# ishine/Test-time-adaptation-ASR-SUTA

Measured on AMD Instinct MI355X. Metric: adapted utterances/sec (whole node) at 10 SUTA steps, w2v2-base; WER parity, higher is better.
Workload: dtype f32; 1 GPU; wav2vec2-base SUTA 10 steps on 128000-sample (8 s) utterances, 164 utterances per GPU per step, scripts/LS.sh flags; model=wav2vec2-base, global_batch=164, seq_len=399, n_samples=128000, suta_steps=10, parallelism=utterance-sharded x1

## Files before the change

test-time-adaptation-asr-suta_amd/config.py:

```python
from __future__ import annotations

import copy
import json
import os
from typing import List

_BASE = dict(
    hidden_size=768, num_hidden_layers=12, num_attention_heads=12, intermediate_size=3072,
    vocab_size=32, conv_dim=[512] * 7, conv_kernel=[10, 3, 3, 3, 3, 2, 2], conv_stride=[5, 2, 2, 2, 2, 2, 2],
    conv_bias=False, feat_extract_norm="group", do_stable_layer_norm=False,
    num_conv_pos_embeddings=128, num_conv_pos_embedding_groups=16, layer_norm_eps=1e-5,
)

_LARGE = dict(_BASE, hidden_size=1024, num_hidden_layers=24, num_attention_heads=16, intermediate_size=4096,
              conv_bias=True, feat_extract_norm="layer", do_stable_layer_norm=True)

_XLSR_1B = dict(_LARGE, hidden_size=1280, num_hidden_layers=48, num_attention_heads=16, intermediate_size=5120)
_XLSR_2B = dict(_LARGE, hidden_size=1920, num_hidden_layers=48, num_attention_heads=16, intermediate_size=7680)

_TINY_GROUP = dict(_BASE, hidden_size=64, num_hidden_layers=2, num_attention_heads=4, intermediate_size=128,
                   conv_dim=[32] * 7, num_conv_pos_embeddings=16, num_conv_pos_embedding_groups=4)
_TINY_LAYER = dict(_TINY_GROUP, conv_bias=True, feat_extract_norm="layer", do_stable_layer_norm=True)
_TINY_HD80 = dict(_TINY_LAYER, hidden_size=160, num_attention_heads=2, num_conv_pos_embedding_groups=2,
                  intermediate_size=320)
_TINY_HD120 = dict(_TINY_HD80, hidden_size=240)

PRESETS = {
    "facebook/wav2vec2-base-960h": _BASE,
    "wav2vec2-base": _BASE,
    "facebook/wav2vec2-large-960h-lv60": _LARGE,
    "facebook/wav2vec2-large-960h-lv60-self": _LARGE,
    "wav2vec2-large": _LARGE,
    "facebook/wav2vec2-xls-r-1b": _XLSR_1B,
    "wav2vec2-xls-r-1b": _XLSR_1B,
    "facebook/wav2vec2-xls-r-2b": _XLSR_2B,
    "wav2vec2-xls-r-2b": _XLSR_2B,
    "tiny-group": _TINY_GROUP,
    "tiny-layer": _TINY_LAYER,
    "tiny-hd80": _TINY_HD80,
    "tiny-hd120": _TINY_HD120,
}


def head_dim(cfg: dict) -> int:
    return cfg["hidden_size"] // cfg["num_attention_heads"]


def flash_attention_applies(cfg: dict) -> bool:
    d = head_dim(cfg)
    return d == 64 or (64 < d <= 128 and d % 8 == 0)


def get_config(name_or_path: str) -> dict:
    if name_or_path in PRESETS:
        return copy.deepcopy(PRESETS[name_or_path])
    cfg_file = os.path.join(name_or_path, "config.json")
    if os.path.isfile(cfg_file):
        with open(cfg_file) as f:
            raw = json.load(f)
        cfg = copy.deepcopy(_BASE)
        for k in cfg:
            if k in raw:
                cfg[k] = raw[k]
        return cfg
    raise KeyError(f"unknown model '{name_or_path}': not a preset and no config.json found")


def frame_lengths(cfg: dict, n_samples: int) -> List[int]:
    out, L = [], int(n_samples)
    for k, s in zip(cfg["conv_kernel"], cfg["conv_stride"]):
        L = (L - k) // s + 1
        out.append(L)
    return out


def num_frames(cfg: dict, n_samples: int) -> int:
    return frame_lengths(cfg, n_samples)[-1]


def param_shapes(cfg: dict):
    H, C = cfg["hidden_size"], cfg["conv_dim"]
    out = [("wav2vec2.masked_spec_embed", (H,))]
    group = cfg["feat_extract_norm"] == "group"
    for i, (c, k) in enumerate(zip(C, cfg["conv_kernel"])):
        cin = 1 if i == 0 else C[i - 1]
        b = f"wav2vec2.feature_extractor.conv_layers.{i}."
        out.append((b + "conv.weight", (c, cin, k)))
        if cfg["conv_bias"]:
            out.append((b + "conv.bias", (c,)))
        if (group and i == 0) or not group:
            out += [(b + "layer_norm.weight", (c,)), (b + "layer_norm.bias", (c,))]
    fp = "wav2vec2.feature_projection."
    out += [(fp + "layer_norm.weight", (C[-1],)), (fp + "layer_norm.bias", (C[-1],)),
# ... 20 lines not shown
```

test-time-adaptation-asr-suta_amd/csrc/common.h:

```cpp
#pragma once
#include <hip/hip_runtime.h>
#include <stdint.h>
#include <string>

#define SUTA_WAVE 64

typedef float f32x4 __attribute__((ext_vector_type(4)));
typedef float f32x16 __attribute__((ext_vector_type(16)));

__device__ __forceinline__ float gelu_f(float x) {
    return 0.5f * x * (1.0f + erff(x * 0.70710678118654752f));
}
__device__ __forceinline__ float dgelu_f(float x) {
    const float cdf = 0.5f * (1.0f + erff(x * 0.70710678118654752f));
    const float pdf = 0.39894228040143268f * __expf(-0.5f * x * x);
    return cdf + x * pdf;
}

__device__ __forceinline__ float erfc_t(float z, float t, float ez2) {
    float p = 0.17087277f;
    p = fmaf(p, t, -0.82215223f);
    p = fmaf(p, t, 1.48851587f);
    p = fmaf(p, t, -1.13520398f);
    p = fmaf(p, t, 0.27886807f);
    p = fmaf(p, t, -0.18628806f);
    p = fmaf(p, t, 0.09678418f);
    p = fmaf(p, t, 0.37409196f);
    p = fmaf(p, t, 1.00002368f);
    p = fmaf(p, t, -1.26551223f);
    return t * ez2 * __expf(p);
}
__device__ __forceinline__ float gelu_fast(float x) {
    const float z = fabsf(x) * 0.70710678118654752f;
    const float t = __builtin_amdgcn_rcpf(fmaf(0.5f, z, 1.0f));
    const float erfc = erfc_t(z, t, __expf(-z * z));
    return 0.5f * x * (x >= 0.f ? 2.0f - erfc : erfc);
}
__device__ __forceinline__ float dgelu_fast(float x) {
    const float z = fabsf(x) * 0.70710678118654752f;
    const float t = __builtin_amdgcn_rcpf(fmaf(0.5f, z, 1.0f));
    const float e = __expf(-z * z);
    const float erfc = erfc_t(z, t, e);
    const float cdf = 0.5f * (x >= 0.f ? 2.0f - erfc : erfc);
    return cdf + x * (0.39894228040143268f * e);
}

struct SutaSwitches {
    int latched;
    int fast_gelu;
    int flash_fwd_plane;
    int flash_bwd_plane;
    int flash_bf16_img;
    int conv_planes;
    int pre_bf16;
    int conv_z_bf16;
    int dy_planes;
    int conv_dx_planes;
    int fused_conv_ln;
    int flash_fwd_nw;
    int hbx;
    int splitk;
    int hbx_form;
    int ln_rpw;
    int hbx_dbg;
    int fused_delta;
    int hbx_t;
    int hbp_conv;
    int hbt4;
    int epi_fast;
    int loss_wide;
    int f32p;
    int sdpl_wide;
};
void suta_latch_switches();
void set_max_lds_once(const void* fn, size_t bytes, const char* name);
const SutaSwitches& suta_switches();

typedef float f32x2v __attribute__((ext_vector_type(2)));
__device__ __forceinline__ f32x2v phi_as2(f32x2v x, f32x2v& q) {
    const f32x2v z = __builtin_elementwise_abs(x) * 0.70710678118654752f;
    f32x2v p = z * 0.0000430638f + 0.0002765672f;
    p = p * z + 0.0001520143f;
    p = p * z + 0.0092705272f;
    p = p * z + 0.0422820123f;
    p = p * z + 0.0705230784f;
    p = p * z + 1.0f;
    p = p * p;
    p = p * p;
    p = p * p;
    p = p * p;
    q = f32x2v{__builtin_amdgcn_rcpf(p.x), __builtin_amdgcn_rcpf(p.y)};
    const f32x2v h = 0.5f * q;
    return f32x2v{x.x >= 0.f ? 1.0f - h.x : h.x, x.y >= 0.f ? 1.0f - h.y : h.y};
}
__device__ __forceinline__ f32x2v gelu2_bf16ep(f32x2v x) {
    f32x2v q;
    return x * phi_as2(x, q);
}
__device__ __forceinline__ f32x2v dgelu2_bf16ep(f32x2v x) {
    f32x2v q;
    const f32x2v cdf = phi_as2(x, q);
    const f32x2v a = x * x * (-0.5f * 1.4426950408889634f);
    const f32x2v e = f32x2v{__builtin_amdgcn_exp2f(a.x), __builtin_amdgcn_exp2f(a.y)};
    return cdf + (x * 0.39894228040143268f) * e;
}

__device__ __forceinline__ float wave_sum(float v) {
#pragma unroll
    for (int o = 32; o > 0; o >>= 1) v += __shfl_xor(v, o, 64);
    return v;
}
__device__ __forceinline__ double wave_sum_d(double v) {
#pragma unroll
    for (int o = 32; o > 0; o >>= 1) v += __shfl_xor(v, o, 64);
    return v;
}
__device__ __forceinline__ float wave_max(float v) {
#pragma unroll
    for (int o = 32; o > 0; o >>= 1) v = fmaxf(v, __shfl_xor(v, o, 64));
    return v;
}

enum {
    EPI_BIAS = 1,
    EPI_GELU = 2,
// ... 16 lines not shown
    long sA0, sA1, sB0, sB1, sC0, sC1;
    int ta, tb;
    int segK, pad, Mvalid;
    int segB;
    long sBseg;
    const float* bias;
    long sBias0, sBias1;
    const float* R;
    long ldr, sR0, sR1;
    const float* aux;
    long ldaux, sAux0, sAux1;
    float* C2;
    long ldc2, sC20, sC21;
    const float* rowv;
    long sRow0, sRow1;
    const int* zrows;
    const int* zmvalid;
    float alpha;
    int epi;
    int splits, kchunk;
    float* ws;
    int va, vb;
    int mode;
    int order;
    const void* Ab;
    const void* Bb;
    long ldab, ldbb;
    void* Cb;
    long ldcb;
    long sCb1;
    int off32;
    int preb;
    int fgelu;
    const float* dlt_o;
    long ldo;
    float* delta;
    int dT, dNH;
};

void gemm_init(GemmParams& p);
bool gemm_hbx_t_selected(const GemmParams& p);
void gemm_launch(GemmParams p, hipStream_t st, float* ws, long ws_floats);
void gemm_set_variant(int tile, int nbuf);
void gemm_set_mode(int mode);
bool gemm_run_hb_class(const GemmParams& p, dim3 grid, hipStream_t st);
void launch_to_bf16(const float* src, long lds, long rows, int K, void* dst, hipStream_t st);
void launch_transpose_bf16(const float* src, long zs, int Z, int K, int N, void* dst, hipStream_t st,
                          void* dstn = nullptr);
int gemm_get_mode();
void gemm_census_enable(bool on);
std::string gemm_census_text();
bool gemm_census_is_on();
void gemm_census_time(const std::string& shape, double ms);
```

test-time-adaptation-asr-suta_amd/csrc/gemm.hip:

```cpp
#include "gemm_kernels.h"
#include <algorithm>
#include <cstdio>
#include <cstdlib>
#include <atomic>
#include <map>
#include <mutex>
#include <stdexcept>
#include <string>

namespace {

bool aligned16(const void* q) { return (reinterpret_cast<uintptr_t>(q) & 15) == 0; }

int g_force_tile = -1;
int g_nbuf = 3;
int g_mode = 0;

}

void gemm_set_variant(int tile, int nbuf) {
    g_force_tile = tile;
    g_nbuf = nbuf;
}

static std::mutex g_census_mu;
static std::map<std::string, long> g_census;
static std::atomic<bool> g_census_on{false};
static std::map<std::string, std::pair<double, long>> g_census_ms;

void gemm_census_enable(bool on) {
    std::lock_guard<std::mutex> lk(g_census_mu);
    g_census_on = on;
    g_census.clear();
    g_census_ms.clear();
}

bool gemm_census_is_on() { return g_census_on; }

void gemm_census_time(const std::string& shape, double ms) {
    std::lock_guard<std::mutex> lk(g_census_mu);
    auto& e = g_census_ms[shape];
    e.first += ms;
    e.second += 1;
}

std::string gemm_census_text() {
    std::lock_guard<std::mutex> lk(g_census_mu);
    std::string out;
    for (const auto& kv : g_census) out += kv.first + " " + std::to_string(kv.second) + "\n";
    for (const auto& kv : g_census_ms)
        out += "ms|" + kv.first + "|n=" + std::to_string(kv.second.second) + " " +
               std::to_string((long)(kv.second.first * 1000.0)) + "\n";
    return out;
}

static void census(const char* kernel, int BM, int BN, const GemmParams& p, int splits) {
    if (!g_census_on) return;
    char key[160], gkey[160], ekey[96];
    snprintf(key, sizeof key, "%s %dx%d z=%ld split=%d %s%s%s", kernel, BM, BN, (long)p.Z, splits, p.ta ? "T" : "N",
             p.tb ? "T" : "N", p.segK > 0 ? (p.segB ? " conv-seg" : " conv") : "");
    snprintf(gkey, sizeof gkey, "grid %s %dx%d gx=%d gy=%d z=%ld split=%d", kernel, BM, BN, (p.N + BN - 1) / BN,
             (p.M + BM - 1) / BM, (long)p.Z, splits);
    snprintf(ekey, sizeof ekey, "epi %s %dx%d %d", kernel, BM, BN, p.epi);
    std::lock_guard<std::mutex> lk(g_census_mu);
    ++g_census[key];
    ++g_census[gkey];
    ++g_census[ekey];
}

void gemm_set_mode(int mode) { g_mode = mode; }
int gemm_get_mode() { return g_mode; }

void gemm_init(GemmParams& p) {
    p = GemmParams{};
    p.Z = 1;
    p.zdiv = 1;
    p.alpha = 1.f;
    p.splits = 1;
    p.mode = g_mode;
}

static int choose_tile(long M, long N, long Z, long K, int mode) {
    struct Cand {
        int bm, bn;
        double eff;
    };
    static const Cand glds[4] = {{128, 128, 1.0}, {128, 64, 0.93}, {64, 128, 0.92}, {64, 64, 0.85}};
    static const Cand x6[4] = {{128, 128, 1.0}, {128, 64, 0.9}, {64, 128, 0.9}, {64, 64, 0.75}};
    const Cand* cands = mode == 0 ? glds : x6;
    int best = 0;
    double bt = 1e300;
    for (int c = 0; c < 4; ++c) {
        const long tiles = ((M + cands[c].bm - 1) / cands[c].bm) * ((N + cands[c].bn - 1) / cands[c].bn) * Z;
        const double area = (double)cands[c].bm * cands[c].bn;
        const double t = std::max((double)tiles, 256.0) * area / cands[c].eff;
        if (t < bt * 0.999) {
// ... 221 lines not shown
```

test-time-adaptation-asr-suta_amd/csrc/ops.h:

```cpp
#pragma once
#include "common.h"

void launch_wave_normalize(const float* x, float* y, int B, long N, const int* lens, hipStream_t st);

void launch_conv0(const float* x, long N, const float* W, const float* bias, long wstride, float* z, int B, int L0,
                  int C, int K, int S, hipStream_t st, void* zb = nullptr);

void launch_front_gn_fwd(const float* x, long N, const float* W, const float* bias, long wstride, int B, int L0, int C,
                         int K, int S, const float* g, const float* beta, float* mean, float* rstd, float* a,
                         double* dpart, const int* L0s, hipStream_t st);
void launch_front_gn_bwd(const float* x, long N, const float* W, const float* bias, long wstride, int B, int L0, int C,
                         int K, int S, const float* g, const float* beta, const float* mean, const float* rstd,
                         float* da, float* dgamma, float* dbeta, float* dW, long gstride, double* dpart, float* fpart,
                         const int* L0s, hipStream_t st);

void launch_layernorm_fwd(const float* x, const float* g, const float* beta, long pstride, int rows_per_utt,
                          float* y, float* xhat, float* rstd, int rows, int D, float eps, int gelu_out,
                          hipStream_t st, void* yb = nullptr, float* mean = nullptr, const void* xb = nullptr);
void launch_layernorm_bwd(const float* dy, const float* xhat, const float* rstd, const float* g, const float* beta,
                          long pstride, int rows_per_utt, int B, int D, int gelu_in, const float* post_aux,
                          const float* resid, float* dx, float* dgamma, float* dbeta, long gstride, float* part,
                          hipStream_t st, void* dxb = nullptr, const float* x = nullptr, const float* mean = nullptr,
                          const void* dyb = nullptr);

long layernorm_bwd_conv_part_floats(int B, int rows_per_utt, int D, int ktaps);
bool launch_layernorm_bwd_conv(const float* dy, const float* rstd, const float* g, const float* beta, long pstride,
                               int rows_per_utt, int B, int D, float* dx, float* dgamma, float* dbeta, float* dbias,
                               float* dw, long gstride, float* part, hipStream_t st, const float* x, const float* mean,
                               const float* xw, long xws, int xs, int ktaps, void* dxb = nullptr, int bf16_in = 0);
void launch_colsum(const float* x, int B, int rows, int C, float* out, long ostride, float* part, hipStream_t st);

bool flash_dh_ok(int dh);
long flash_dq_scratch_floats(int B, int T, int NH, int dh);
bool flash_fwd_reads_plane(bool bf16, const void* qkvb, int H, int dh);
bool flash_bwd_reads_planes(bool bf16, const void* qkvb, const void* dctxb, int H, int dh);
bool launch_flash_fwd(const float* qkv, float* ctx, float* lse, int B, int T, int NH, int H, int dh, float scale,
                      const int* tlen, bool bf16, hipStream_t st, void* ctxb = nullptr, const void* qkvb = nullptr);
bool launch_flash_bwd(const float* qkv, const float* dctx, const float* lse, const float* delta, float* dqkv,
                      float* dqp, int B, int T, int NH, int H, int dh, float scale, const int* tlen, bool bf16,
                      hipStream_t st, void* dqkvb = nullptr, const void* qkvb = nullptr,
                      const void* dctxb = nullptr);
bool flash_wide_dh(int dh);
long flash_wide_dq_scratch_floats(int B, int T, int NH, int dh);
bool launch_flash_wide_fwd(const float* qkv, float* ctx, float* lse, int B, int T, int NH, int H, int dh, float scale,
                           const int* tlen, bool bf16, hipStream_t st, void* ctxb);
bool launch_flash_wide_bwd(const float* qkv, const float* dctx, const float* lse, const float* delta, float* dqkv,
                           float* dqp, int B, int T, int NH, int H, int dh, float scale, const int* tlen, bool bf16,
                           hipStream_t st, void* dqkvb);
bool launch_posconv(bool fwd, const float* x, const float* W, const float* bias, const float* R, float* C, float* C2,
                    int B, int T, int H, int G, int K, int pad, const int* tlen, hipStream_t st);
bool launch_posconv_bf16(bool fwd, const float* x, const void* Wt, const float* bias, const float* R, float* C,
                         float* C2, int B, int T, int H, int G, int K, int pad, const int* tlen, hipStream_t st);
void launch_softmax_rows(float* s, long nrows, int T, long ld, const int* tlen, long rows_per_utt, hipStream_t st);

void launch_attn_delta(const float* dO, const float* O, float* delta, int B, int T, int NH, int dh, hipStream_t st);

void launch_dgelu_mul(const float* g, const float* z, float* out, long n, hipStream_t st);

struct LossHP {
    float temp, em_coef, div_coef;
    int reweight, non_blank;
};
#define SUTA_MAX_VOCAB 1024
size_t suta_loss_scratch_floats(int B, long T, int V);
void launch_suta_loss(const float* logits, int B, int T, int V, LossHP hp, const int* tlen, float* dlogits, float* loss,
                      float* scratch, hipStream_t st);

enum { SDPL_KIND_NORMAL = 0, SDPL_KIND_DROP = 1, SDPL_KIND_SPACE = 2, SDPL_KIND_FAIL = 3 };
enum { SDPL_FLAG_LOOKUP = 1, SDPL_FLAG_INFEASIBLE = 2 };
struct SdplTable {
    const int* off;
    const int* ids;
    const int* kind;
    int space_id;
};
long sdpl_scratch_floats(int T, int V);
void launch_sdpl_loss(const float* logits, int B, int T, int V, float pl_coef, const int* tlen, float* dlogits,
                      float* loss, float* scratch, int* err, const SdplTable* tab, hipStream_t st);

void launch_argmax(const float* logits, long rows, int V, int* ids, hipStream_t st);

struct AdamRun {
    long start, len;
    int k;
};
#define SUTA_MAX_RUNS 24
#define ADAM_TAB 52
struct AdamArgs {
    int nruns;
    AdamRun runs[SUTA_MAX_RUNS];
    int blk0[SUTA_MAX_RUNS];
    float beta1, beta2, omb1, omb2, eps, lr_wd;
    int sgd;
    float step_size[5][5];
    float bc2_sqrt[5][5];
    const float* tab;
    const int* step;
};
void launch_broadcast(float* dst, const float* src, long n, int B, hipStream_t st);
void launch_step_advance(int* step, hipStream_t st);
void launch_adam(float* P, const float* G, float* M, float* V, long pstride, int B, const AdamArgs& a,
                 hipStream_t st);
```

test-time-adaptation-asr-suta_amd/csrc/ops.hip:

```cpp
#include "ops.h"
#include <algorithm>
#include <map>
#include <mutex>
#include <stdexcept>
#include <string>

namespace {

inline int cdiv(long a, long b) { return (int)((a + b - 1) / b); }

template <typename T>
__device__ __forceinline__ T block_sum(T v, T* red) {
    const int lane = threadIdx.x & 63, w = threadIdx.x >> 6;
#pragma unroll
    for (int o = 32; o > 0; o >>= 1) v += __shfl_xor(v, o, 64);
    __syncthreads();
    if (lane == 0) red[w] = v;
    __syncthreads();
    T s = red[0] + red[1] + red[2] + red[3];
    __syncthreads();
    return s;
}

__global__ __launch_bounds__(256) void wave_normalize_kernel(const float* __restrict__ x, float* __restrict__ y,
                                                             long N, const int* __restrict__ lens) {
    __shared__ double red[4];
    const float* xb = x + (long)blockIdx.x * N;
    float* yb = y + (long)blockIdx.x * N;
    const long n = lens ? lens[blockIdx.x] : N;
    double s = 0.0;
    for (long i = threadIdx.x; i < n; i += 256) s += xb[i];
    s = block_sum(s, red);
    const double mean = s / (double)n;
    double q = 0.0;
    for (long i = threadIdx.x; i < n; i += 256) {
        const double d = (double)xb[i] - mean;
        q += d * d;
    }
    q = block_sum(q, red);
    const float meanf = (float)mean;
    const float denom = (float)sqrt(q / (double)n + 1e-7);
    for (long i = threadIdx.x; i < N; i += 256) yb[i] = i < n ? (xb[i] - meanf) / denom : 0.f;
}

constexpr int C0_ROWS = 32;
__global__ __launch_bounds__(256) void conv0_kernel(const float* __restrict__ x, long N, const float* __restrict__ W,
                                                    const float* __restrict__ bias, long wstride,
                                                    float* __restrict__ z, int L0, int C, int K, int S) {
    __shared__ float xs[C0_ROWS * 16 + 16];
    const int b = blockIdx.y;
    const int t0 = blockIdx.x * C0_ROWS;
    const float* xb = x + (long)b * N;
    const float* Wb = W + (long)b * wstride;
    const float* bb = bias ? bias + (long)b * wstride : nullptr;
    const int nx = (C0_ROWS - 1) * S + K;
    for (int i = threadIdx.x; i < nx; i += 256) {
        const long gi = (long)t0 * S + i;
        xs[i] = gi < N ? xb[gi] : 0.f;
// ... 778 lines not shown
                const int row = (it * 4) / CG, col = (it * 4) % CG;
                *reinterpret_cast<f32x4*>(dst + row * WS + col) = st[n];
            }
        }
    };
    f32x4 acc[NC];
#pragma unroll
    for (int nf = 0; nf < NC; ++nf) acc[nf] = f32x4{0.f, 0.f, 0.f, 0.f};
    const int nch = K / CHT;
    load_chunk(0);
    store_chunk(0);
    __syncthreads();
    const float* arow = win + (16 * w + r) * XS + g;
    for (int c = 0; c < nch; ++c) {
        if (c + 1 < nch) load_chunk(c + 1);
        const float* wb = wbuf + (c & 1) * (CHT * CG * WS) + g * WS + r;
#pragma unroll
        for (int qq = 0; qq < CHT; ++qq) {
            const float* ap = arow + (c * CHT + qq) * XS;
            const float* bp = wb + qq * CG * WS;
#pragma unroll
            for (int j = 0; j < CG / 4; ++j) {
                const float a = ap[4 * j];
                float b[NC];
#pragma unroll
                for (int nf = 0; nf < NC; ++nf) b[nf] = bp[4 * j * WS + 16 * nf];
#pragma unroll
                for (int nf = 0; nf < NC; ++nf) acc[nf] = __builtin_amdgcn_mfma_f32_16x16x4f32(a, b[nf], acc[nf], 0, 0, 0);
            }
        }
        if (c + 1 < nch) store_chunk((c + 1) & 1);
        __syncthreads();
    }
#pragma unroll
    for (int i = 0; i < 4; ++i) {
        const int t = t0 + 16 * w + 4 * g + i;
        if (t >= T) continue;
        const long o = ((long)u * T + t) * H + gi * CG;
#pragma unroll
        for (int nf = 0; nf < NC; ++nf) {
            const int co = 16 * nf + r;
            float v;
            if (FWD) {
                v = acc[nf][i] * 1.0f + bias[gi * CG + co];
                C2[o + co] = v;
                v = gelu_f(v) + R[o + co];
            } else {
                v = acc[nf][i] + R[o + co];
                if (tlen && t >= tl) v = 0.f;
            }
            C[o + co] = v;
        }
    }
}

constexpr int PCB_CHT = 4;
constexpr int PCB_RS = 72;
template <int WB, bool FWD>
__global__ __launch_bounds__(WB * 64, 1) void posconv_bf16_kernel(const float* __restrict__ x,
                                                                  const __bf16* __restrict__ Wt,
                                                                  const float* __restrict__ bias,
                                                                  const float* __restrict__ R, float* __restrict__ C,
                                                                  float* __restrict__ C2, int T, int H, int G, int K,
                                                                  int pad, const int* __restrict__ tlen, int ntile,
                                                                  int nutt) {
    constexpr int CG = 64, NT = WB * 64, WROWS = 32 * WB;
    constexpr int CHUNK = PCB_CHT * CG * CG / 8;
    constexpr int LPT = (CHUNK + NT - 1) / NT;
    extern __shared__ __attribute__((aligned(16))) __bf16 pcb_smem[];
    __bf16* win = pcb_smem;
    __bf16* wbuf = pcb_smem + (WROWS + K - 1) * PCB_RS;
    typedef __bf16 b8 __attribute__((ext_vector_type(8)));
    typedef __bf16 b4 __attribute__((ext_vector_type(4)));

    const int nb = gridDim.x;
    int L = blockIdx.x;
    if ((nb & 7) == 0) L = (L & 7) * (nb >> 3) + (L >> 3);
    const int tile = L % ntile;
    const int u = (L / ntile) % nutt;
    const int gi = L / (ntile * nutt);
    const int t0 = tile * WROWS;
    const int tl = tlen ? tlen[u] : T;
    const int w = threadIdx.x >> 6, lane = threadIdx.x & 63, l32 = lane & 31, h = lane >> 5;
    const float* xb = x + (long)u * T * H + gi * CG;
    const __bf16* wg = Wt + (long)gi * K * CG * CG;

    const int nwin = (WROWS + K - 1) * (CG / 4);
    for (int it = threadIdx.x; it < nwin; it += NT) {
        const int row = it / (CG / 4), c4 = (it % (CG / 4)) * 4;
        const int t = t0 - pad + row;
        f32x4 v = {0.f, 0.f, 0.f, 0.f};
        if (t >= 0 && t < tl) v = *reinterpret_cast<const f32x4*>(xb + (long)t * H + c4);
        b4 o;
#pragma unroll
        for (int e = 0; e < 4; ++e) o[e] = (__bf16)v[e];
        *reinterpret_cast<b4*>(win + row * PCB_RS + c4) = o;
    }
    b8 st[LPT];
    auto load_chunk = [&](int c) {
        const b8* src = reinterpret_cast<const b8*>(wg + (long)c * PCB_CHT * CG * CG);
#pragma unroll
        for (int n = 0; n < LPT; ++n) {
            const int it = threadIdx.x + n * NT;
            if (it < CHUNK) st[n] = src[it];
        }
    };
// ... 944 lines not shown
#undef LBC
    const int nvec = 3 + ktaps;
    hipLaunchKernelGGL(chunk_reduce_conv, dim3(cdiv(D, 256), B, nvec), dim3(256), 0, st, part, nchunk, nvec, D, dgamma,
                       dbeta, dbias, dw, gstride);
    return true;
}

void launch_colsum(const float* x, int B, int rows, int C, float* out, long ostride, float* part, hipStream_t st) {
    const int nchunk = cdiv(rows, CS_ROWS);
    hipLaunchKernelGGL(colsum_partial, dim3(nchunk, B), dim3(256), 0, st, x, rows, C, part, nchunk);
    hipLaunchKernelGGL(chunk_reduce, dim3(cdiv(C, 256), B), dim3(256), 0, st, part, nchunk, 1, C, out, (float*)nullptr,
                       ostride);
}

void launch_softmax_rows(float* s, long nrows, int T, long ld, const int* tlen, long rows_per_utt, hipStream_t st) {
    dim3 grid((unsigned)((nrows + 3) / 4));
    if (T <= 256) hipLaunchKernelGGL(softmax_rows_kernel<4>, grid, dim3(256), 0, st, s, nrows, T, ld, tlen,
                                    rows_per_utt);
    else if (T <= 512) hipLaunchKernelGGL(softmax_rows_kernel<8>, grid, dim3(256), 0, st, s, nrows, T, ld, tlen,
                                    rows_per_utt);
    else if (T <= 1024) hipLaunchKernelGGL(softmax_rows_kernel<16>, grid, dim3(256), 0, st, s, nrows, T, ld, tlen,
                                    rows_per_utt);
    else hipLaunchKernelGGL(softmax_rows_kernel<32>, grid, dim3(256), 0, st, s, nrows, T, ld, tlen,
                                    rows_per_utt);
}

constexpr int PC_CHT = 2;
#define HIPCHK_OPS(x)                                                                        \
    do {                                                                                     \
        if ((x) != hipSuccess) throw std::runtime_error("hipFuncSetAttribute(posconv) failed"); \
    } while (0)

template <int CG, bool FWD>
static void posconv_go(int WB, dim3 grid, size_t lds, hipStream_t st, const float* x, const float* W,
                       const float* bias, const float* R, float* C, float* C2, int T, int H, int G, int K, int pad,
                       const int* tlen, int ntile, int B) {
#define PC(WB_)                                                                                                   \
    do {                                                                                                          \
        set_max_lds_once(reinterpret_cast<const void*>(&posconv_kernel<CG, WB_, PC_CHT, FWD>), 160 * 1024,       \
                         "posconv_kernel");                                                                       \
        hipLaunchKernelGGL((posconv_kernel<CG, WB_, PC_CHT, FWD>), grid, dim3(WB_ * 64), lds, st, x, W, bias, R, C, \
                           C2, T, H, G, K, pad, tlen, ntile, B);                                                  \
    } while (0)
    switch (WB) {
        case 4: PC(4); break;
        case 5: PC(5); break;
        case 6: PC(6); break;
        case 7: PC(7); break;
        default: PC(8); break;
    }
#undef PC
}

bool launch_posconv(bool fwd, const float* x, const float* W, const float* bias, const float* R, float* C, float* C2,
                    int B, int T, int H, int G, int K, int pad, const int* tlen, hipStream_t st) {
    const int CG = H / G;
    if ((CG != 48 && CG != 64) || K % PC_CHT || H % 4) return false;
    int WB = 8;
    long best = 1L << 40;
    for (int wb = 8; wb >= 4; --wb) {
        const long tiles = (T + 16 * wb - 1) / (16 * wb);
        const long waste = tiles * 16 * wb - T;
        if (waste < best) {
            best = waste;
            WB = wb;
        }
    }
    const int ntile = (T + 16 * WB - 1) / (16 * WB);
    const int XS = CG + 4, WS = (CG % 64 == 0) ? CG + 16 : CG;
    const size_t lds = ((size_t)(16 * WB + K - 1) * XS + 2 * PC_CHT * CG * WS) * sizeof(float);
    if (lds > 160 * 1024) return false;
    const dim3 grid((unsigned)((long)G * B * ntile));
    if (CG == 48) {
        if (fwd) posconv_go<48, true>(WB, grid, lds, st, x, W, bias, R, C, C2, T, H, G, K, pad, tlen, ntile, B);
        else posconv_go<48, false>(WB, grid, lds, st, x, W, bias, R, C, C2, T, H, G, K, pad, tlen, ntile, B);
    } else {
        if (fwd) posconv_go<64, true>(WB, grid, lds, st, x, W, bias, R, C, C2, T, H, G, K, pad, tlen, ntile, B);
        else posconv_go<64, false>(WB, grid, lds, st, x, W, bias, R, C, C2, T, H, G, K, pad, tlen, ntile, B);
    }
    return true;
}

template <bool FWD>
static void posconv_bf16_go(int WB, dim3 grid, size_t lds, hipStream_t st, const float* x, const __bf16* W,
                            const float* bias, const float* R, float* C, float* C2, int T, int H, int G, int K, int pad,
                            const int* tlen, int ntile, int B) {
#define PCB(WB_)                                                                                                  \
    do {                                                                                                          \
        set_max_lds_once(reinterpret_cast<const void*>(&posconv_bf16_kernel<WB_, FWD>), 160 * 1024,              \
                         "posconv_bf16_kernel");                                                                  \
        hipLaunchKernelGGL((posconv_bf16_kernel<WB_, FWD>), grid, dim3(WB_ * 64), lds, st, x, W, bias, R, C, C2, T, \
                           H, G, K, pad, tlen, ntile, B);                                                         \
    } while (0)
    switch (WB) {
        case 4: PCB(4); break;
        case 5: PCB(5); break;
        case 6: PCB(6); break;
        case 7: PCB(7); break;
        default: PCB(8); break;
    }
#undef PCB
}

bool launch_posconv_bf16(bool fwd, const float* x, const void* Wt, const float* bias, const float* R, float* C,
                         float* C2, int B, int T, int H, int G, int K, int pad, const int* tlen, hipStream_t st) {
    if (H / G != 64 || H % G || K % PCB_CHT || !Wt) return false;
    int WB = 8;
    long best = 1L << 40;
    for (int wb = 8; wb >= 4; --wb) {
        const long tiles = (T + 32 * wb - 1) / (32 * wb);
        const long waste = tiles * 32 * wb - T;
        if (waste < best) {
            best = waste;
            WB = wb;
        }
    }
    const int ntile = (T + 32 * WB - 1) / (32 * WB);
    const size_t lds = ((size_t)(32 * WB + K - 1) * PCB_RS + 2 * PCB_CHT * 64 * PCB_RS) * sizeof(__bf16);
    if (lds > 160 * 1024) return false;
    const dim3 grid((unsigned)((long)G * B * ntile));
    const __bf16* W = reinterpret_cast<const __bf16*>(Wt);
    if (fwd) posconv_bf16_go<true>(WB, grid, lds, st, x, W, bias, R, C, C2, T, H, G, K, pad, tlen, ntile, B);
    else posconv_bf16_go<false>(WB, grid, lds, st, x, W, bias, R, C, C2, T, H, G, K, pad, tlen, ntile, B);
    return true;
}
// ... 74 lines not shown
void set_max_lds_once(const void* fn, size_t bytes, const char* name) {
    static std::mutex mu;
    static std::map<const void*, size_t> done;
    std::lock_guard<std::mutex> lk(mu);
    auto it = done.find(fn);
    if (it != done.end() && it->second >= bytes) return;
    if (hipFuncSetAttribute(fn, hipFuncAttributeMaxDynamicSharedMemorySize, (int)bytes) != hipSuccess)
        throw std::runtime_error(std::string("hipFuncSetAttribute(") + name + ") failed");
    done[fn] = bytes;
}

static thread_local SutaSwitches g_switches{};

void suta_latch_switches() {
    auto on = [](const char* name) {
        const char* ev = std::getenv(name);
        return (ev && atoi(ev) == 0) ? 0 : 1;
    };
    SutaSwitches s{};
    s.fast_gelu = on("SUTA_FAST_GELU");
    s.flash_fwd_plane = on("SUTA_FLASH_FWD_PLANE");
    s.flash_bwd_plane = on("SUTA_FLASH_BWD_PLANE");
    s.flash_bf16_img = on("SUTA_FLASH_BF16_IMG");
    s.conv_planes = on("SUTA_CONV_PLANES");
    s.pre_bf16 = on("SUTA_PRE_BF16");
    s.conv_z_bf16 = on("SUTA_CONV_Z_BF16");
    s.dy_planes = on("SUTA_DY_PLANES");
    s.conv_dx_planes = on("SUTA_CONV_DX_PLANES");
    s.fused_conv_ln = on("SUTA_FUSED_CONV_LN");
    const char* hbx = std::getenv("SUTA_HBX");
    s.hbx = hbx ? atoi(hbx) : 1;
    s.splitk = on("SUTA_SPLITK");
    const char* hbxt = std::getenv("SUTA_HBX_T");
    s.hbx_t = hbxt ? std::min(2, std::max(0, atoi(hbxt))) : 2;
    s.fused_delta = on("SUTA_FUSED_DELTA");
    const char* lrpw = std::getenv("SUTA_LN_RPW");
    s.ln_rpw = lrpw ? atoi(lrpw) : 2;
    const char* hform = std::getenv("SUTA_HBX_FORM");
    s.hbx_form = hform ? atoi(hform) : 4;
    const char* ht4 = std::getenv("SUTA_HBT4");
    s.hbt4 = ht4 ? atoi(ht4) : 1;
    const char* hdbg = std::getenv("SUTA_HBX_DBG");
    s.hbx_dbg = hdbg ? atoi(hdbg) : 0;
    const char* fnw = std::getenv("SUTA_FLASH_FWD_NW");
    s.flash_fwd_nw = (fnw && atoi(fnw) == 8) ? 8 : 4;
    s.epi_fast = on("SUTA_EPI_FAST");
    s.hbp_conv = on("SUTA_HBP_CONV");
    const char* lw = std::getenv("SUTA_LOSS_WIDE");
    s.loss_wide = (lw && atoi(lw) != 0) ? 1 : 0;
    const char* f32p = std::getenv("SUTA_F32P");
    s.f32p = f32p ? std::min(2, std::max(0, atoi(f32p))) : 1;
    const char* sw = std::getenv("SUTA_SDPL_WIDE");
    s.sdpl_wide = (sw && atoi(sw) != 0) ? 1 : 0;
    s.latched = 1;
    g_switches = s;
}

const SutaSwitches& suta_switches() {
    if (!g_switches.latched) suta_latch_switches();
    return g_switches;
}

static bool fast_gelu_on() { return suta_switches().fast_gelu != 0; }
template <int MODE, typename... Args>
static void launch_conv0_gn(dim3 grid, hipStream_t st, int K, int S, Args... args) {
    if (K == 10 && S == 5 && fast_gelu_on())
        hipLaunchKernelGGL((conv0_gn_kernel<MODE, 10, 5, true>), grid, dim3(256), 0, st, args...);
    else if (K == 10 && S == 5)
        hipLaunchKernelGGL((conv0_gn_kernel<MODE, 10, 5>), grid, dim3(256), 0, st, args...);
    else
        hipLaunchKernelGGL((conv0_gn_kernel<MODE, 0, 0>), grid, dim3(256), 0, st, args...);
}

void launch_front_gn_fwd(const float* x, long N, const float* W, const float* bias, long wstride, int B, int L0, int C,
                         int K, int S, const float* g, const float* beta, float* mean, float* rstd, float* a,
                         double* dpart, const int* L0s, hipStream_t st) {
    const int nchunk = cdiv(L0, F0_ROWS);
    launch_conv0_gn<0>(dim3(nchunk, B), st, K, S, x, N, W, bias, wstride, L0, C, K, S,
                       (const float*)nullptr, (const float*)nullptr, (const float*)nullptr, (const float*)nullptr,
                       (float*)nullptr, (const float*)nullptr, dpart, (float*)nullptr, nchunk, L0s);
    hipLaunchKernelGGL(col_stats_final, dim3(cdiv(C, 256), B), dim3(256), 0, st, dpart, nchunk, L0, C, 1e-5f, mean,
                       rstd, L0s);
    launch_conv0_gn<1>(dim3(nchunk, B), st, K, S, x, N, W, bias, wstride, L0, C, K, S,
                       mean, rstd, g, beta, a, (const float*)nullptr, (double*)nullptr, (float*)nullptr, nchunk, L0s);
}

void launch_front_gn_bwd(const float* x, long N, const float* W, const float* bias, long wstride, int B, int L0, int C,
                         int K, int S, const float* g, const float* beta, const float* mean, const float* rstd,
                         float* da, float* dgamma, float* dbeta, float* dW, long gstride, double* dpart, float* fpart,
                         const int* L0s, hipStream_t st) {
    const int nchunk = cdiv(L0, F0_ROWS);
    launch_conv0_gn<2>(dim3(nchunk, B), st, K, S, x, N, W, bias, wstride, L0, C, K, S,
                       mean, rstd, g, beta, da, (const float*)nullptr, dpart, (float*)nullptr, nchunk, L0s);
    float* coef = reinterpret_cast<float*>(dpart + (long)B * nchunk * 2 * C);
    hipLaunchKernelGGL(gn_bwd_final, dim3(cdiv(C, 256), B), dim3(256), 0, st, dpart, nchunk, C, dgamma, dbeta, gstride,
                       coef);
    launch_conv0_gn<3>(dim3(nchunk, B), st, K, S, x, N, W, bias, wstride, L0, C, K, S,
                       mean, rstd, g, beta, da, coef, (double*)nullptr, fpart, nchunk, L0s);
    hipLaunchKernelGGL(conv0_dw_reduce, dim3(cdiv((long)K * C, 256), B), dim3(256), 0, st, fpart, nchunk, K * C, dW,
                       gstride);
}

void launch_attn_delta(const float* dO, const float* O, float* delta, int B, int T, int NH, int dh, hipStream_t st) {
    const long items = (long)B * T * NH;
    const long vec = items * (dh / 4);
    const dim3 grid((unsigned)((vec + 255) / 256));
// ... 19 lines not shown
```

Before: 39.08 utt/s.

## Add load-balanced positional-conv kernel that splits time tiles across idle CUs

Adds a posconv_bal kernel plus a cost-model planner that picks between the existing time-tiled positional convolution and a balanced grid. The balanced grid splits each (group, utterance) pair into several time blocks and spreads the leftover pairs across spare CUs so the last wave is not mostly idle, with an XCD-aware split by 8. The planner uses the CU count and chooses the balanced path only when its estimated cost is not worse, and it is on by default (SUTA_POSCONV_BAL=1). The trade-off is re-reading the K-1 halo rows for every extra time block, plus added complexity in the planner logic.

```diff
diff --git a/test-time-adaptation-asr-suta_amd/config.py b/test-time-adaptation-asr-suta_amd/config.py
--- a/test-time-adaptation-asr-suta_amd/config.py
+++ b/test-time-adaptation-asr-suta_amd/config.py
@@ -24,6 +24,9 @@
 _TINY_HD80 = dict(_TINY_LAYER, hidden_size=160, num_attention_heads=2, num_conv_pos_embedding_groups=2,
                   intermediate_size=320)
 _TINY_HD120 = dict(_TINY_HD80, hidden_size=240)
+_TINY_PC48 = dict(_TINY_LAYER, hidden_size=96, num_attention_heads=2, intermediate_size=192,
+                  num_conv_pos_embeddings=128, num_conv_pos_embedding_groups=2)
+_TINY_PC64 = dict(_TINY_PC48, hidden_size=128, intermediate_size=256)
 
 PRESETS = {
     "facebook/wav2vec2-base-960h": _BASE,
@@ -39,6 +42,8 @@
     "tiny-layer": _TINY_LAYER,
     "tiny-hd80": _TINY_HD80,
     "tiny-hd120": _TINY_HD120,
+    "tiny-pc48": _TINY_PC48,
+    "tiny-pc64": _TINY_PC64,
 }
 
 
diff --git a/test-time-adaptation-asr-suta_amd/csrc/common.h b/test-time-adaptation-asr-suta_amd/csrc/common.h
--- a/test-time-adaptation-asr-suta_amd/csrc/common.h
+++ b/test-time-adaptation-asr-suta_amd/csrc/common.h
@@ -71,6 +71,7 @@
     int loss_wide;
     int f32p;
     int sdpl_wide;
+    int posconv_bal;
 };
 void suta_latch_switches();
 void set_max_lds_once(const void* fn, size_t bytes, const char* name);
@@ -193,3 +194,4 @@
 std::string gemm_census_text();
 bool gemm_census_is_on();
 void gemm_census_time(const std::string& shape, double ms);
+void gemm_census_note(const std::string& key);
diff --git a/test-time-adaptation-asr-suta_amd/csrc/gemm.hip b/test-time-adaptation-asr-suta_amd/csrc/gemm.hip
--- a/test-time-adaptation-asr-suta_amd/csrc/gemm.hip
+++ b/test-time-adaptation-asr-suta_amd/csrc/gemm.hip
@@ -42,6 +42,12 @@
     auto& e = g_census_ms[shape];
     e.first += ms;
     e.second += 1;
+}
+
+void gemm_census_note(const std::string& key) {
+    if (!g_census_on) return;
+    std::lock_guard<std::mutex> lk(g_census_mu);
+    ++g_census[key];
 }
 
 std::string gemm_census_text() {
diff --git a/test-time-adaptation-asr-suta_amd/csrc/ops.h b/test-time-adaptation-asr-suta_amd/csrc/ops.h
--- a/test-time-adaptation-asr-suta_amd/csrc/ops.h
+++ b/test-time-adaptation-asr-suta_amd/csrc/ops.h
@@ -49,6 +49,18 @@
                            hipStream_t st, void* dqkvb);
 bool launch_posconv(bool fwd, const float* x, const float* W, const float* bias, const float* R, float* C, float* C2,
                     int B, int T, int H, int G, int K, int pad, const int* tlen, hipStream_t st);
+struct PosconvPlan {
+    bool ok, bal;
+    int WB, ntile;
+    long grid, cost;
+    size_t lds;
+    int bal_waves;
+    int gp_nx, gp_pairs_x, gp_full_x, gp_nblk_a, gp_nblk_b, gp_nft;
+    long bal_grid, bal_cost;
+    size_t bal_lds;
+};
+PosconvPlan posconv_plan(int B, int T, int H, int G, int K);
+std::string posconv_plan_text(const PosconvPlan& p, int CG);
 bool launch_posconv_bf16(bool fwd, const float* x, const void* Wt, const float* bias, const float* R, float* C,
                          float* C2, int B, int T, int H, int G, int K, int pad, const int* tlen, hipStream_t st);
 void launch_softmax_rows(float* s, long nrows, int T, long ld, const int* tlen, long rows_per_utt, hipStream_t st);
diff --git a/test-time-adaptation-asr-suta_amd/csrc/ops.hip b/test-time-adaptation-asr-suta_amd/csrc/ops.hip
--- a/test-time-adaptation-asr-suta_amd/csrc/ops.hip
+++ b/test-time-adaptation-asr-suta_amd/csrc/ops.hip
@@ -1,9 +1,11 @@
 #include "ops.h"
 #include <algorithm>
+#include <atomic>
 #include <map>
 #include <mutex>
 #include <stdexcept>
 #include <string>
+#include <type_traits>
 
 namespace {
 
@@ -888,6 +890,153 @@
             C[o + co] = v;
         }
     }
+}
+
+struct PcBalGrid {
+    int nx, pairs_x, full_x, nblk_a, nblk_b, nft;
+};
+
+template <int CG, int NWV, int TPW, int CHT, bool FWD>
+__global__ __launch_bounds__(NWV * 64, 1) void posconv_bal_kernel(const float* __restrict__ x,
+                                                                  const float* __restrict__ W,
+                                                                  const float* __restrict__ bias,
+                                                                  const float* __restrict__ R, float* __restrict__ C,
+                                                                  float* __restrict__ C2, int T, int H, int K, int pad,
+                                                                  const int* __restrict__ tlen, int nutt,
+                                                                  PcBalGrid gp) {
+    constexpr int NT = NWV * 64, NC = CG / 16, XS = PcLayout<CG>::XS, WS = PcLayout<CG>::WS;
+    constexpr int CHUNK4 = CHT * CG * CG / 4;
+    constexpr int LPT = (CHUNK4 + NT - 1) / NT;
+    extern __shared__ __attribute__((aligned(16))) float pc_smem[];
+
+    const int xp = blockIdx.x % gp.nx, l = blockIdx.x / gp.nx;
+    const int na = gp.full_x * gp.nblk_a;
+    int pl, kb, nblk;
+    if (l < na) {
+        pl = l / gp.nblk_a, kb = l % gp.nblk_a, nblk = gp.nblk_a;
+    } else {
+        pl = gp.full_x + (l - na) / gp.nblk_b, kb = (l - na) % gp.nblk_b, nblk = gp.nblk_b;
+    }
+    const int pair = xp * gp.pairs_x + pl;
+    const int gi = pair / nutt, u = pair % nutt;
+    const int tq = gp.nft / nblk, trem = gp.nft % nblk;
+    const int ft0 = kb * tq + min(kb, trem);
+    const int nb = tq + (kb < trem ? 1 : 0);
+    const int t0 = ft0 * 16;
+    const int wrows = 16 * nb + K - 1;
+    float* win = pc_smem;
+    float* wbuf = pc_smem + wrows * XS;
+
+    const int tl = tlen ? tlen[u] : T;
+    const int w = threadIdx.x >> 6, lane = threadIdx.x & 63;
+    const int r = lane & 15, g = lane >> 4;
+    const float* xb = x + (long)u * T * H + gi * CG;
+    const float* wg = W + (long)gi * K * CG * CG;
+
+    const int nwin = wrows * (CG / 4);
+    for (int it = threadIdx.x; it < nwin; it += NT) {
+        const int row = it / (CG / 4), c4 = (it % (CG / 4)) * 4;
+        const int t = t0 - pad + row;
+        f32x4 v = {0.f, 0.f, 0.f, 0.f};
+        if (t >= 0 && t < tl) v = *reinterpret_cast<const f32x4*>(xb + (long)t * H + c4);
+        *reinterpret_cast<f32x4*>(win + row * XS + c4) = v;
+    }
+    f32x4 st[LPT];
+    auto load_chunk = [&](int c) {
+        const float* src = wg + (long)c * CHT * CG * CG;
+#pragma unroll
+        for (int n = 0; n < LPT; ++n) {
+            const int it = threadIdx.x + n * NT;
+            st[n] = it < CHUNK4 ? *reinterpret_cast<const f32x4*>(src + it * 4) : f32x4{0.f, 0.f, 0.f, 0.f};
+        }
+    };
+    auto store_chunk = [&](int buf) {
+        float* dst = wbuf + buf * (CHT * CG * WS);
+#pragma unroll
+        for (int n = 0; n < LPT; ++n) {
+            const int it = threadIdx.x + n * NT;
+            if (it < CHUNK4) {
+                const int row = (it * 4) / CG, col = (it * 4) % CG;
+                *reinterpret_cast<f32x4*>(dst + row * WS + col) = st[n];
+            }
+        }
+    };
+    const int nch = K / CHT;
+    load_chunk(0);
+    store_chunk(0);
+    __syncthreads();
+    const float* arow = win + (16 * w + r) * XS + g;
+
+    auto run = [&](auto ntag) {
+        constexpr int N = decltype(ntag)::value;
+        f32x4 acc[N > 0 ? N : 1][NC];
+#pragma unroll
+        for (int i = 0; i < N; ++i)
+#pragma unroll
+            for (int nf = 0; nf < NC; ++nf) acc[i][nf] = f32x4{0.f, 0.f, 0.f, 0.f};
+        for (int c = 0; c < nch; ++c) {
+            if (c + 1 < nch) load_chunk(c + 1);
+            const float* wb = wbuf + (c & 1) * (CHT * CG * WS) + g * WS + r;
+#pragma unroll
+            for (int qq = 0; qq < CHT; ++qq) {
+                const float* ap = arow + (c * CHT + qq) * XS;
+                const float* bp = wb + qq * CG * WS;
+#pragma unroll
+                for (int j = 0; j < CG / 4; ++j) {
+                    float a[N > 0 ? N : 1], b[NC];
+#pragma unroll
+                    for (int i = 0; i < N; ++i) a[i] = ap[16 * NWV * i * XS + 4 * j];
+#pragma unroll
+                    for (int nf = 0; nf < NC; ++nf) b[nf] = bp[4 * j * WS + 16 * nf];
+#pragma unroll
+                    for (int i = 0; i < N; ++i)
+#pragma unroll
+                        for (int nf = 0; nf < NC; ++nf)
+                            acc[i][nf] = __builtin_amdgcn_mfma_f32_16x16x4f32(a[i], b[nf], acc[i][nf], 0, 0, 0);
+                }
+            }
+            if (c + 1 < nch) store_chunk((c + 1) & 1);
+            __syncthreads();
+        }
+#pragma unroll
+        for (int i = 0; i < N; ++i) {
+#pragma unroll
+            for (int ii = 0; ii < 4; ++ii) {
+                const int t = t0 + 16 * (w + NWV * i) + 4 * g + ii;
+                if (t >= T) continue;
+                const long o = ((long)u * T + t) * H + gi * CG;
+#pragma unroll
+                for (int nf = 0; nf < NC; ++nf) {
+                    const int co = 16 * nf + r;
+                    float v;
+                    if (FWD) {
+                        v = acc[i][nf][ii] * 1.0f + bias[gi * CG + co];
+                        C2[o + co] = v;
+                        v = gelu_f(v) + R[o + co];
+                    } else {
+                        v = acc[i][nf][ii] + R[o + co];
+                        if (tlen && t >= tl) v = 0.f;
+                    }
+                    C[o + co] = v;
+                }
+            }
+        }
+    };
+    const int nmine = w < nb ? (nb - w + NWV - 1) / NWV : 0;
+    static_assert(TPW >= 1 && TPW <= 4, "tiles per wave");
+#define PCBAL_RUN(N_)                                                   \
+    case N_:                                                          \
+        if constexpr (N_ <= TPW) run(std::integral_constant<int, N_>{}); \
+        break;
+    switch (nmine) {
+        PCBAL_RUN(0)
+        PCBAL_RUN(1)
+        PCBAL_RUN(2)
+        PCBAL_RUN(3)
+        PCBAL_RUN(4)
+        default: break;
+    }
+#undef PCBAL_RUN
 }
 
 constexpr int PCB_CHT = 4;
@@ -1938,10 +2087,34 @@
 #undef PC
 }
 
-bool launch_posconv(bool fwd, const float* x, const float* W, const float* bias, const float* R, float* C, float* C2,
-                    int B, int T, int H, int G, int K, int pad, const int* tlen, hipStream_t st) {
-    const int CG = H / G;
-    if ((CG != 48 && CG != 64) || K % PC_CHT || H % 4) return false;
+template <int CG, int NWV, int TPW, bool FWD>
+static void posconv_bal_go(dim3 grid, size_t lds, hipStream_t st, const float* x, const float* W, const float* bias,
+                           const float* R, float* C, float* C2, int T, int H, int K, int pad, const int* tlen, int B,
+                           const PcBalGrid& gp) {
+    set_max_lds_once(reinterpret_cast<const void*>(&posconv_bal_kernel<CG, NWV, TPW, PC_CHT, FWD>), 160 * 1024,
+                     "posconv_bal_kernel");
+    hipLaunchKernelGGL((posconv_bal_kernel<CG, NWV, TPW, PC_CHT, FWD>), grid, dim3(NWV * 64), lds, st, x, W, bias, R, C,
+                       C2, T, H, K, pad, tlen, B, gp);
+}
+
+static int posconv_cu_count() {
+    static std::atomic<int> ncu{0};
+    int n = ncu.load();
+    if (n > 0) return n;
+    int dev = 0;
+    if (hipGetDevice(&dev) != hipSuccess ||
+        hipDeviceGetAttribute(&n, hipDeviceAttributeMultiprocessorCount, dev) != hipSuccess || n < 8)
+        n = 256;
+    ncu.store(n);
+    return n;
+}
+
+PosconvPlan posconv_plan(int B, int T, int H, int G, int K) {
+    PosconvPlan p{};
+    const int CG = G > 0 ? H / G : 0;
+    if (G <= 0 || H % G || (CG != 48 && CG != 64) || K % PC_CHT || H % 4 || B < 1 || T < 1) return p;
+    const int XS = CG + 4, WS = (CG % 64 == 0) ? CG + 16 : CG;
+    const int ncu = posconv_cu_count();
     int WB = 8;
     long best = 1L << 40;
     for (int wb = 8; wb >= 4; --wb) {
@@ -1952,11 +2125,78 @@
             WB = wb;
         }
     }
-    const int ntile = (T + 16 * WB - 1) / (16 * WB);
-    const int XS = CG + 4, WS = (CG % 64 == 0) ? CG + 16 : CG;
-    const size_t lds = ((size_t)(16 * WB + K - 1) * XS + 2 * PC_CHT * CG * WS) * sizeof(float);
-    if (lds > 160 * 1024) return false;
-    const dim3 grid((unsigned)((long)G * B * ntile));
+    p.WB = WB;
+    p.ntile = (T + 16 * WB - 1) / (16 * WB);
+    p.lds = ((size_t)(16 * WB + K - 1) * XS + 2 * PC_CHT * CG * WS) * sizeof(float);
+    p.grid = (long)G * B * p.ntile;
+    p.ok = p.lds <= 160 * 1024;
+    p.cost = ((p.grid + ncu - 1) / ncu) * ((WB + 3) / 4);
+    const int mode = suta_switches().posconv_bal;
+    const int cap = CG == 48 ? 28 : 8;
+    const int nft = (T + 15) / 16;
+    const int nblk_a = (nft + cap - 1) / cap;
+    const int tb = (nft + nblk_a - 1) / nblk_a;
+    const size_t lds_b = ((size_t)(16 * tb + K - 1) * XS + 2 * PC_CHT * CG * WS) * sizeof(float);
+    const long pairs = (long)G * B;
+    const int nx = (G % 8 == 0 && ncu % 8 == 0) ? 8 : 1;
+    const int pairs_x = (int)(pairs / nx), ncu_x = ncu / nx;
+    int full_x = pairs_x, nblk_b = 1;
+    long cost_b;
+    if (mode != 3 && nblk_a == 1 && pairs_x % ncu_x && std::min(ncu_x / (pairs_x % ncu_x), nft) > 1) {
+        full_x = pairs_x / ncu_x * ncu_x;
+        nblk_b = std::min(ncu_x / (pairs_x - full_x), nft);
+        const int tb_b = (nft + nblk_b - 1) / nblk_b;
+        cost_b = (long)(full_x / ncu_x) * ((tb + 3) / 4) + (tb_b + 3) / 4;
+    } else {
+        cost_b = (((long)pairs_x * nblk_a + ncu_x - 1) / ncu_x) * ((tb + 3) / 4);
+    }
+    p.bal_cost = cost_b;
+    p.bal_lds = lds_b;
+    p.bal_waves = 8;
+    p.gp_nx = nx, p.gp_pairs_x = pairs_x, p.gp_full_x = full_x, p.gp_nblk_a = nblk_a, p.gp_nblk_b = nblk_b;
+    p.gp_nft = nft;
+    p.bal_grid = (long)nx * ((long)full_x * nblk_a + (long)(pairs_x - full_x) * nblk_b);
+    const bool bal_ok = lds_b <= 160 * 1024 && p.bal_grid < (1L << 31);
+    const long cost_w = tb >= 2 * p.bal_waves ? cost_b * 7 : cost_b * 8;
+    p.bal = mode != 0 && bal_ok && (!p.ok || cost_w <= p.cost * 8 || mode >= 2);
+    if (p.bal) p.ok = true;
+    return p;
+}
+
+std::string posconv_plan_text(const PosconvPlan& p, int CG) {
+    char key[160];
+    if (!p.ok) return "posconv none";
+    if (p.bal)
+        snprintf(key, sizeof key, "posconv bal cg=%d waves=%d nft=%d nblk=%d tail=%d grid=%ld cost=%ld/%ld", CG, p.bal_waves,
+                 p.gp_nft, p.gp_nblk_a, p.gp_nblk_b, p.bal_grid, p.bal_cost, p.cost);
+    else
+        snprintf(key, sizeof key, "posconv wb cg=%d waves=%d ntile=%d grid=%ld cost=%ld/%ld", CG, p.WB, p.ntile, p.grid,
+                 p.cost, p.bal_cost);
+    return key;
+}
+
+bool launch_posconv(bool fwd, const float* x, const float* W, const float* bias, const float* R, float* C, float* C2,
+                    int B, int T, int H, int G, int K, int pad, const int* tlen, hipStream_t st) {
+    const PosconvPlan p = posconv_plan(B, T, H, G, K);
+    if (!p.ok) return false;
+    const int CG = H / G;
+    if (gemm_census_is_on()) gemm_census_note(posconv_plan_text(p, CG));
+    if (p.bal) {
+        const PcBalGrid gp{p.gp_nx, p.gp_pairs_x, p.gp_full_x, p.gp_nblk_a, p.gp_nblk_b, p.gp_nft};
+        const dim3 grid((unsigned)p.bal_grid);
+#define PCBAL(CG_, NWV_, TPW_)                                                                                        \
+    do {                                                                                                              \
+        if (fwd) posconv_bal_go<CG_, NWV_, TPW_, true>(grid, p.bal_lds, st, x, W, bias, R, C, C2, T, H, K, pad, tlen, B, gp); \
+        else posconv_bal_go<CG_, NWV_, TPW_, false>(grid, p.bal_lds, st, x, W, bias, R, C, C2, T, H, K, pad, tlen, B, gp);    \
+    } while (0)
+        if (CG == 48) PCBAL(48, 8, 4);
+        else PCBAL(64, 8, 1);
+#undef PCBAL
+        return true;
+    }
+    const int WB = p.WB, ntile = p.ntile;
+    const size_t lds = p.lds;
+    const dim3 grid((unsigned)p.grid);
     if (CG == 48) {
         if (fwd) posconv_go<48, true>(WB, grid, lds, st, x, W, bias, R, C, C2, T, H, G, K, pad, tlen, ntile, B);
         else posconv_go<48, false>(WB, grid, lds, st, x, W, bias, R, C, C2, T, H, G, K, pad, tlen, ntile, B);
@@ -2137,6 +2377,8 @@
     s.f32p = f32p ? std::min(2, std::max(0, atoi(f32p))) : 1;
     const char* sw = std::getenv("SUTA_SDPL_WIDE");
     s.sdpl_wide = (sw && atoi(sw) != 0) ? 1 : 0;
+    const char* pcb = std::getenv("SUTA_POSCONV_BAL");
+    s.posconv_bal = pcb ? std::min(3, std::max(0, atoi(pcb))) : 1;
     s.latched = 1;
     g_switches = s;
 }
```

After: 39.40 utt/s (median of 6 runs). About the same (+0.8%).
